# young-how/DQN-based-UAV-3D_path_planer

Hardware: NVIDIA H100
Metric: env steps/sec (+ DQN updates/sec), 500x500x100 city (higher is better)
Workload: dtype f64 env state / f32 obs+learner

## Files before the change

### dqn-based-uav-3d_path_planer_b200/csrc/learner.cu

```cuda
#include "learner.cuh"
#include "mlp_tile.cuh"
#include "tc_forward.cuh"

#include <math.h>
#include <string.h>

#include <string>
#include <vector>

namespace uavrl {

int build_mlp(int in_dim, int n_hidden, const int32_t *hidden, int head_main, int head_extra, NetDev &n)
{
    memset(&n, 0, sizeof(n));
    if (in_dim <= 0 || in_dim > kMaxDim) return fail(UAVRL_ERR_INVALID, "in_dim must be in [1,128]");
    if (n_hidden < 1 || n_hidden > UAVRL_MAX_HIDDEN) return fail(UAVRL_ERR_INVALID, "n_hidden must be in [1,4]");
    if (head_main < 1 || head_main + head_extra > 32) return fail(UAVRL_ERR_INVALID, "head width must be in [1,32]");
    n.in_dim = in_dim; n.n_actions = head_main; n.dueling = 0;
    n.n_layers = n_hidden + 1;
    int in = in_dim, poff = 0, soff = 0;
    for (int l = 0; l < n.n_layers; ++l) {
        LayerDev &L = n.L[l];
        const bool head = (l == n_hidden);
        const int out_real = head ? head_main : hidden[l];
// ... 522 lines not shown
        if (l->cfg.algo != UAVRL_ALGO_DQN) {
            a.img = l->tc_img_local; a.mode = kTcArgmax;
            if ((rc = launch_tc_forward(l, a, st))) return rc;
            a.mode = kTcTdGather;
        } else {
            a.mode = kTcTdMax;
        }
        a.img = l->tc_img_target;
        if ((rc = launch_tc_forward(l, a, st))) return rc;
        y_in = l->y_buf;
    }
    if (mid) UAVRL_CUDA(cudaEventRecord(mid[0], st));
    int nparts = grid, n_loss_parts = grid;
    AdamArgs a;
    memset(&a, 0, sizeof(a));
    a.P = l->net.P; a.apply = apply ? 1 : 0; a.world = l->world;
    a.img_floats = l->net.smem_w_floats; a.tc_floats = l->tc.train_img_bytes / 4;
    a.inv_b = 1.0f / (float)global_batch;
    if (apply && !partials_only) {
        adam_hyper(a, l->cfg.lr, ++l->adam_t);
        a.hard = hard_update_due(l);
    }
    if (y_in && l->tc_train_ok) {
        if (B > l->train_cap) {
            UAVRL_CUDA(cudaStreamSynchronize(st));
            cudaFree(l->act_buf); cudaFree(l->dz_buf);
            UAVRL_CUDA(cudaMalloc((void **)&l->act_buf, (size_t)l->G * B * (size_t)(l->tc.act_stride > 0 ? l->tc.act_stride : 4) * 4));
            UAVRL_CUDA(cudaMalloc((void **)&l->dz_buf, (size_t)l->G * B * (size_t)l->tc.dz_stride * 4));
            l->train_cap = B;
        }
        int rc = launch_tc_train(l, src, B, global_batch, y_in, &nparts, &n_loss_parts, st, mid ? mid[1] : nullptr, fuse_td);
        if (rc) return rc;
    } else {
    UpdateArgs ua;
    ua.img_local = l->img_local; ua.img_target = l->img_target; ua.partials = l->partials; ua.loss_partials = l->loss_partials;
    ua.B = B; ua.n_tiles = n_tiles; ua.algo = l->cfg.algo; ua.gamma = l->cfg.gamma; ua.dual = l->dual_weights;
    ua.loss_kind = l->cfg.loss_kind; ua.img_floats = l->net.smem_w_floats;
    ua.inv_global_b = 1.0f / (float)global_batch;
    ua.y_in = y_in;
    update_kernel<<<dim3(grid, l->G), kNetThreads, upd_smem_bytes(l->net, l->dual_weights), st>>>(l->net, src, ua);
    l->pdl_prev = kPdlNone;
    UAVRL_LAUNCHED();
    if (mid) UAVRL_CUDA(cudaEventRecord(mid[1], st));
    }
    if (mid) UAVRL_CUDA(cudaEventRecord(mid[2], st));
    l->last_nparts = nparts;
    l->last_n_loss_parts = n_loss_parts;
    l->last_global_batch = global_batch;
    if (partials_only) {
        if (per_batch) return per_set(l, B, l->per.idx, nullptr, l->per.abs_err, 1, st);
        return 0;
    }
    a.nparts = nparts; a.n_loss_parts = n_loss_parts;
// ... 454 lines not shown
```

### dqn-based-uav-3d_path_planer_b200/csrc/tc_chain.cuh

```cuda
#pragma once
#include "tc_forward.cuh"
#include "tma.cuh"
#include "wgmma.cuh"

namespace uavrl {

__device__ __forceinline__ void stage_trace(long long *t, int slot)
{
    if (t && blockIdx.x == 0 && blockIdx.y == 0 && threadIdx.x == 0) t[slot] = clock64();
}

template <class RowOf>
__device__ __forceinline__ void a0_load(const RowOf &row_of, int i0, int R, int in_dim, int K0, float4 (&v)[4])
{
    const int total = R * (K0 / 4), lgR = 31 - __clz(R);
#pragma unroll
    for (int u = 0; u < 4; ++u) {
        const int i = i0 + u * kTcThreads;
        const int r = i & (R - 1), j = i >> lgR;
        const float *rp = (i < total) ? row_of(r) : nullptr;
        v[u] = (rp && 4 * j < in_dim) ? __ldg(reinterpret_cast<const float4 *>(rp) + j) : make_float4(0.f, 0.f, 0.f, 0.f);
    }
}
__device__ __forceinline__ void a0_load_sel(const float *const *rows, const uint8_t *fresh, bool want_fresh, int R, int in_dim, int K0, float4 (&v)[4])
{
    const int total = R * (K0 / 4), lgR = 31 - __clz(R);
#pragma unroll
    for (int u = 0; u < 4; ++u) {
        const int i = threadIdx.x + u * kTcThreads;
        const int r = i & (R - 1), j = i >> lgR;
        const float *rp = (i < total) ? rows[r] : nullptr;
        const bool take = rp && 4 * j < in_dim && ((fresh[r] != 0) == want_fresh);
        if (!want_fresh) v[u] = take ? __ldg(reinterpret_cast<const float4 *>(rp) + j) : make_float4(0.f, 0.f, 0.f, 0.f);
        else if (take) v[u] = __ldcg(reinterpret_cast<const float4 *>(rp) + j);
    }
}
__device__ __forceinline__ void a0_store(const float4 (&v)[4], int i0, int R, int K0, unsigned char *Ahi, unsigned char *Alo)
{
    const int total = R * (K0 / 4), lgR = 31 - __clz(R);
    const uint32_t sbo = mma_sbo(K0);
#pragma unroll
    for (int u = 0; u < 4; ++u) {
        const int i = i0 + u * kTcThreads;
        if (i < total) {
            const int r = i & (R - 1), j = i >> lgR;
            float4 h, l;
            tf32_split(v[u].x, h.x, l.x); tf32_split(v[u].y, h.y, l.y); tf32_split(v[u].z, h.z, l.z); tf32_split(v[u].w, h.w, l.w);
            const uint32_t off = mma_off(r, 4 * j, sbo);
            *reinterpret_cast<float4 *>(Ahi + off) = h;
            *reinterpret_cast<float4 *>(Alo + off) = l;
        }
    }
}
template <class RowOf>
__device__ __forceinline__ void a0_gather(const RowOf &row_of, int R, int in_dim, int K0, unsigned char *Ahi, unsigned char *Alo)
{
    for (int i0 = threadIdx.x; i0 < R * (K0 / 4); i0 += 4 * kTcThreads) {
        float4 v[4];
        a0_load(row_of, i0, R, in_dim, K0, v);
        a0_store(v, i0, R, K0, Ahi, Alo);
    }
}

template <bool KEEP>
__device__ __forceinline__ uint32_t hidden_epilogue(const EpiSlice &e, const float *acc, int acc_ld, const float *bias, int N,
                                                    unsigned char *Ahi, unsigned char *Alo, float *act_row, bool mine)
{
    const uint32_t sbon = mma_sbo(N);
    uint32_t mk = 0u;
    for (int c = e.c0, sh = 0; c < N; c += e.step, sh += 4) {
        const float4 v = e.ld(acc, acc_ld, c);
        float4 x, h, lo4;
        x.x = fmaxf(v.x + bias[c + 0], 0.f); x.y = fmaxf(v.y + bias[c + 1], 0.f);
        x.z = fmaxf(v.z + bias[c + 2], 0.f); x.w = fmaxf(v.w + bias[c + 3], 0.f);
        tf32_split(x.x, h.x, lo4.x); tf32_split(x.y, h.y, lo4.y); tf32_split(x.z, h.z, lo4.z); tf32_split(x.w, h.w, lo4.w);
        const uint32_t off = mma_off(e.row, c, sbon);
        *reinterpret_cast<float4 *>(Ahi + off) = h;
        *reinterpret_cast<float4 *>(Alo + off) = lo4;
        if (KEEP) {
            if (mine) *reinterpret_cast<float4 *>(act_row + c) = x;
            mk |= ((x.x > 0.f ? 1u : 0u) | (x.y > 0.f ? 2u : 0u) | (x.z > 0.f ? 4u : 0u) | (x.w > 0.f ? 8u : 0u)) << sh;
        }
    }
    return mine ? mk : 0u;
}

template <bool DUELING>
__device__ __forceinline__ void q_combine(const float *bias, int nA, float (&q)[32])
{
#pragma unroll
    for (int j = 0; j < 32; ++j) q[j] += bias[j];
    if (DUELING) {
        float s = 0.f, V = 0.f;
#pragma unroll
        for (int j = 0; j < 32; ++j) { if (j < nA) s += q[j]; if (j == nA) V = q[j]; }
        const float mean = s / (float)nA;
#pragma unroll
        for (int j = 0; j < 32; ++j) q[j] = V + q[j] - mean;
    }
}
template <bool DUELING>
__device__ __forceinline__ void q_row(const float *acc, int acc_ld, int row, const float *bias, int nA, float (&q)[32])
{
// ... 7 lines not shown
#pragma unroll
    for (int j = 1; j < 32; ++j) if (j < nA && q[j] > bv) { bv = q[j]; best = j; }
    return best;
}
__device__ __forceinline__ float q_at(const float (&q)[32], int a)
{
    float v = 0.f;
#pragma unroll
    for (int j = 0; j < 32; ++j) if (j == a) v = q[j];
    return v;
}

__device__ __forceinline__ uint32_t fwd_image_split(const TcNet &tc) { return tc.n_layers > 1 ? (uint32_t)tc.L[1].hi_off : (uint32_t)tc.img_bytes; }
__device__ __forceinline__ void stage_forward_image(const TcNet &tc, unsigned char *W, const unsigned char *img, uint64_t *wbar, uint64_t *wbar2)
{
    const uint32_t split = fwd_image_split(tc);
    fence_proxy_async();
    bulk_g2s_chunked(W, img, split, wbar);
    if (split < (uint32_t)tc.img_bytes) bulk_g2s_chunked(W + split, img + split, (uint32_t)tc.img_bytes - split, wbar2);
}

template <bool FIXED, bool KEEP, class Mid, class Head, class Done>
__device__ __forceinline__ void forward_layers(const TcNet &tc, int R, const EpiSlice &e, unsigned char *Ahi, unsigned char *Alo,
                                               const unsigned char *W, float *acc, float *act_row, bool mine, Mid &&mid, Head &&head,
                                               Done &&done)
{
    const float *bias_all = reinterpret_cast<const float *>(W + tc.bias_base);
    for (int l = 0; l < tc.n_layers; ++l) {
        const TcLayer T = tc.L[l];
        mma_3xtf32<kMmaFwd, FIXED>(acc, tc.acc_ld, Ahi, Alo, W + T.hi_off, W + T.lo_off, mma_sbo(T.K_pad), T.N_pad, T.K_pad / 8, R);
        mid(l);
        const float *bias = bias_all + T.bias_off;
        if (l + 1 < tc.n_layers) {
            const uint32_t mk = hidden_epilogue<KEEP>(e, acc, tc.acc_ld, bias, T.N_pad, Ahi, Alo, KEEP ? act_row + tc.L[l + 1].act_off : nullptr, mine);
            fence_proxy_async();
            __syncthreads();
            done(l, mk);
        } else {
            head(l, bias);
        }
    }
}

}
```

### dqn-based-uav-3d_path_planer_b200/csrc/tc_forward.cu

```cuda
#include <stdarg.h>
#include <stdlib.h>
#include <string.h>

#include "tc_chain.cuh"

namespace uavrl {

static inline int rup(int x, int m) { return (x + m - 1) / m * m; }

size_t tc_smem_bytes(const TcNet &tc) { return (size_t)2 * tc.a_bytes + (size_t)tc.img_bytes + (size_t)tc.max_rows * tc.acc_ld * 4; }

int tc_build(const uavrl_learner_config &c, const NetDev &net, TcNet &tc, std::vector<int32_t> &hi_map, std::vector<int32_t> &lo_map,
             std::vector<int32_t> &hi2_map, std::vector<int32_t> &lo2_map)
{
    memset(&tc, 0, sizeof(tc));
    tc.n_layers = net.n_layers; tc.in_dim = net.in_dim; tc.n_actions = net.n_actions; tc.dueling = net.dueling;
    if (net.in_dim % 4 != 0) return -1;
    int off = 0, maxK = 0, k_pad = rup(net.in_dim, 8);
    for (int l = 0; l < net.n_layers; ++l) {
        const LayerDev &L = net.L[l];
        TcLayer &T = tc.L[l];
        const bool head = (l == net.n_layers - 1);
        T.K_real = L.in; T.K_pad = k_pad; T.N_real = L.out;
        T.N_pad = head ? 32 : rup(L.out, 16);
// ... 14 lines not shown
    for (int l = 0; l < net.n_layers; ++l) {
        TcLayer &T = tc.L[l];
        T.t_hi_off = T.t_lo_off = -1;
        if (l == 0) continue;
        const int bytes = T.K_pad * T.N_pad * 4;
        T.t_hi_off = toff; toff += bytes;
        T.t_lo_off = toff; toff += bytes;
    }
    tc.train_img_bytes = rup(toff, 16);
    tc.max_k = maxK;
    {
        int maxN = 32;
        for (int l = 0; l < net.n_layers; ++l) if (tc.L[l].N_pad > maxN) maxN = tc.L[l].N_pad;
        tc.acc_ld = rup(maxN, 32) + 4;
    }
    tc.max_rows = kTcTile;
    tc.a_bytes = (int)mma_tile_bytes(tc.max_rows, maxK);
    if (tc_smem_bytes(tc) + 4096 > 227 * 1024) {
        tc.max_rows = 64;
        tc.a_bytes = (int)mma_tile_bytes(tc.max_rows, maxK);
    }
    int ao = 0, dzo = 0;
    for (int l = 0; l < net.n_layers; ++l) {
        tc.L[l].act_off = (l == 0) ? -1 : ao;
        if (l > 0) ao += tc.L[l].K_pad;
        tc.L[l].dz_off = dzo; dzo += tc.L[l].N_pad;
    }
    tc.act_stride = ao; tc.dz_stride = dzo;
    hi_map.assign((size_t)net.P, -1); lo_map.assign((size_t)net.P, -1);
    hi2_map.assign((size_t)net.P, -1); lo2_map.assign((size_t)net.P, -1);
    auto elem = [](int k_pad_cols, int base, int n, int k) {
        const int sbo = (k_pad_cols / 4) * 128;
        return (base + (n >> 3) * sbo + (k >> 2) * 128 + (n & 7) * 16 + (k & 3) * 4) / 4;
    };
    for (int l = 0; l < net.n_layers; ++l) {
        const LayerDev &L = net.L[l];
        const TcLayer &T = tc.L[l];
        const int out_main = T.out_main;
        for (int o = 0; o < L.out; ++o) {
            const bool vrow = (o >= out_main);
            for (int k = 0; k < L.in; ++k) {
                const size_t pi = vrow ? (size_t)L.w2_off + (size_t)(o - out_main) * L.in + k : (size_t)L.w_off + (size_t)o * L.in + k;
                hi_map[pi] = elem(T.K_pad, T.hi_off, o, k);
                lo_map[pi] = elem(T.K_pad, T.lo_off, o, k);
                if (l > 0) {
                    hi2_map[pi] = elem(T.N_pad, T.t_hi_off, k, o);
                    lo2_map[pi] = elem(T.N_pad, T.t_lo_off, k, o);
                }
// ... 297 lines not shown
```

### dqn-based-uav-3d_path_planer_b200/csrc/tc_train.cu

```cuda
#include <string.h>
#include <stdlib.h>

#include <atomic>

#include "tc_chain.cuh"

namespace uavrl {

constexpr int kDwChunk = 128;

struct TcTrainArgs {
    const unsigned char *img;
    BatchSrc src;
    int32_t B, R, n_tiles;
    const float *y;
    float inv_global_b;
    float *act_buf, *dz_buf;
    float *loss_partials;
    int32_t loss_kind;
    int32_t fused_td, algo;
    float gamma;
    const unsigned char *img_target;
    int64_t img_stride;
    long long *trace;
};

struct TcDwArgs {
    BatchSrc src;
    int32_t B, n_chunks, P;
    int32_t n_slices;
    const float *act_buf, *dz_buf;
    float *partials;
    long long *trace;
};

template <int NPRE, bool DUELING, bool FIXED>
__global__ void __launch_bounds__(kTcThreads, 1) tc_train_kernel(TcNet tc, TcTrainArgs a)
{
    stage_trace(a.trace, 0);
    extern __shared__ __align__(1024) unsigned char smem[];
    const int R = a.R;
    const uint32_t a_bytes = (uint32_t)(R / 8) * mma_sbo(tc.max_k);
    unsigned char *Ahi = smem, *Alo = smem + a_bytes, *W = smem + 2 * a_bytes;
    float *acc = reinterpret_cast<float *>(W + tc.train_img_bytes);
    __shared__ uint64_t wbar, wbar2, wbar3;
    __shared__ const float *rows[kTcTile];
    __shared__ const float *rows2[kTcTile];
    __shared__ int s_act[kTcTile], s_astar[kTcTile];
    __shared__ uint8_t s_fresh[kTcTile];
    __shared__ float s_y[kTcTile], s_rew[kTcTile], s_done[kTcTile];
    __shared__ float s_loss[4];

    const int tid = threadIdx.x, warp = tid >> 5, lane = tid & 31, quad = warp & 3, half = warp >> 2;
    const int grp = blockIdx.y;
    const unsigned char *img = a.img + (size_t)grp * (size_t)a.img_stride, *img_t = a.img_target + (size_t)grp * (size_t)a.img_stride;
    const BatchSrc src = trainer_src(a.src, grp, a.B, tc.in_dim);
    const size_t r0 = (size_t)grp * (size_t)a.B;
    float *act_buf = a.act_buf + r0 * tc.act_stride, *dz_buf = a.dz_buf + r0 * tc.dz_stride;
    const float *y_in = a.y ? a.y + r0 : nullptr;
    constexpr int kCtl = kTcThreads - 32;
    if (tid == 0) s_loss[0] = s_loss[1] = s_loss[2] = s_loss[3] = 0.f;
    constexpr bool fused = NPRE > 0;
    constexpr int n_pre = NPRE;
    uint32_t wphase = 0;
    if (tid == kCtl) {
        mbar_init(&wbar, 1); mbar_init(&wbar2, 1); mbar_init(&wbar3, 1); fence_barrier_init();
        fence_proxy_async();
        if (!fused) bulk_g2s_chunked(W, img, (uint32_t)tc.train_img_bytes, &wbar);
        else {
            bulk_g2s_chunked(W, (n_pre == 2) ? img : img_t, (uint32_t)tc.img_bytes, &wbar);
            if (tc.train_img_bytes > tc.img_bytes)
                bulk_g2s_chunked(W + tc.img_bytes, img + tc.img_bytes, (uint32_t)(tc.train_img_bytes - tc.img_bytes), &wbar3);
        }
    }
    stage_trace(a.trace, 1);
    bool waited = false;

    uint32_t pkey[4];
    Philox::gen(src.key, src.epoch, 0x5A17ull, pkey);
    bool wready = false;
    const int nl = tc.n_layers;
    const int row = quad * 32 + lane;
    const bool live = quad * 32 < R;
    const EpiSlice e(R, kTcThreads);
    uint32_t hm1 = 0u, hm2 = 0u, hm3 = 0u, hm4 = 0u;
    const auto table = [](const float *const *t) { return [t](int r) { return t[r]; }; };

    for (int tile = blockIdx.x; tile < a.n_tiles; tile += gridDim.x) {
        const int base = tile * R;
        int64_t my_slot = -1;
        if (tid < R) {
            const int b = base + tid;
            const float *p = nullptr, *p2 = nullptr;
            bool fr = false;
            if (b < a.B) my_slot = resolve_rows(src, b, tc.in_dim, pkey, p, p2, &fr);
            rows[tid] = p;
            if (fused) { rows2[tid] = p2; s_astar[tid] = 0; s_fresh[tid] = fr ? 1 : 0; }
        }
        __syncthreads();
        const bool early_rows = n_pre > 0 && R * (tc.L[0].K_pad / 4) <= 4 * kTcThreads;
        float4 vmain[4], vnext[4];
        if (early_rows) {
            a0_load_sel(rows2, s_fresh, false, R, tc.in_dim, tc.L[0].K_pad, vnext);
            a0_load(table(rows), tid, R, tc.in_dim, tc.L[0].K_pad, vmain);
        }
        if (fused && !waited) { pdl_wait(); pdl_trigger(); waited = true; }
        int m_act = 0; float m_rew = 0.f, m_done = 0.f;
        if (my_slot >= 0) load_meta(src, my_slot, m_act, m_rew, m_done);
        if (early_rows) a0_load_sel(rows2, s_fresh, true, R, tc.in_dim, tc.L[0].K_pad, vnext);
        auto park_meta = [&]() { if (tid < R) { s_act[tid] = m_act; if (fused) { s_rew[tid] = m_rew; s_done[tid] = m_done; } } };
        stage_trace(a.trace, 2);
        for (int pass = 0; pass < n_pre; ++pass) {
// ... 5 lines not shown
            else a0_gather(table(rows2), R, tc.in_dim, tc.L[0].K_pad, Ahi, Alo);
            if (pass == 0) { park_meta(); stage_trace(a.trace, 3); }
            mbar_wait(&wbar, wphase); wphase ^= 1;
            fence_proxy_async();
            __syncthreads();
            if (pass == 0) stage_trace(a.trace, 4);
            const bool td_pass = (pass == n_pre - 1);
            const auto head = [&](int l, const float *bias) {
                if (half == 0 && live) {
                    float q[32], bv;
                    q_row<DUELING>(acc, tc.acc_ld, row, bias, tc.n_actions, q);
                    const int best = q_argmax(q, tc.n_actions, bv);
                    if (!td_pass) s_astar[row] = best;
                    else s_y[row] = td_target(s_rew[row], a.gamma, n_pre == 2 ? q_at(q, s_astar[row]) : bv, s_done[row]);
                }
                fence_proxy_async();
                __syncthreads();
                if (pass == 0) stage_trace(a.trace, 5 + l);
            };
            forward_layers<FIXED, false>(tc, R, e, Ahi, Alo, W, acc, nullptr, false, [](int) {}, head,
                                         [&](int l, uint32_t) { if (pass == 0) stage_trace(a.trace, 5 + l); });
        }
        if (fused && tid == kCtl) stage_forward_image(tc, W, img, &wbar, &wbar2);
        if (early_rows) a0_store(vmain, tid, R, tc.L[0].K_pad, Ahi, Alo);
        else a0_gather(table(rows), R, tc.in_dim, tc.L[0].K_pad, Ahi, Alo);
        stage_trace(a.trace, 9);
        if (!waited) { pdl_wait(); pdl_trigger(); waited = true; }
        if (n_pre == 0) park_meta();
        if (!fused && tid < R) s_y[tid] = (base + tid < a.B) ? y_in[base + tid] : 0.f;
        if (fused) { mbar_wait(&wbar, wphase); wphase ^= 1; }
        else if (!wready) { mbar_wait(&wbar, 0); wready = true; }
        fence_proxy_async();
        __syncthreads();
        stage_trace(a.trace, 10);
        const int gb = base + row;
        const bool mine = live && gb < a.B;
        const int egb = base + e.row;
        const bool emine = egb < a.B;

        const auto mid = [&](int l) {
            if (fused && l == 0 && fwd_image_split(tc) < (uint32_t)tc.img_bytes) mbar_wait(&wbar2, 0);
            if (l < 4) stage_trace(a.trace, 27 + l);
        };
        const auto head = [&](int l, const float *bias) {
            const TcLayer &T = tc.L[l];
            if (half == 0 && live) {
                const int nA = tc.n_actions;
                float q[32];
// ... 1 lines not shown
                stage_trace(a.trace, 21);
                q_combine<DUELING>(bias, nA, q);
                const int act = s_act[row];
                const float qa = q_at(q, act);
                stage_trace(a.trace, 22);
                float gq = 0.f, lterm = 0.f;
                if (mine) lterm = td_loss(src, gb, qa - s_y[row], a.loss_kind, a.inv_global_b, gq);
#pragma unroll
                for (int off = 16; off > 0; off >>= 1) lterm += __shfl_xor_sync(0xffffffffu, lterm, off);
                stage_trace(a.trace, 23);
                if (lane == 0) s_loss[quad] += lterm;
                stage_trace(a.trace, 24);
                float g[32];
                const float inv = 1.f / (float)nA;
#pragma unroll
                for (int j = 0; j < 32; ++j) {
                    float gj;
                    if (DUELING) gj = (j < nA) ? gq * ((j == act ? 1.f : 0.f) - inv) : (j == nA ? gq : 0.f);
                    else gj = (j == act) ? gq : 0.f;
                    g[j] = gj;
                }
                stage_trace(a.trace, 25);
                const uint32_t sbon = mma_sbo(T.N_pad);
                float *dz_row = dz_buf + (size_t)gb * tc.dz_stride + T.dz_off;
#pragma unroll
                for (int j = 0; j < 8; ++j) {
                    float4 x = make_float4(g[4 * j], g[4 * j + 1], g[4 * j + 2], g[4 * j + 3]), h, lo4;
                    tf32_split(x.x, h.x, lo4.x); tf32_split(x.y, h.y, lo4.y); tf32_split(x.z, h.z, lo4.z); tf32_split(x.w, h.w, lo4.w);
                    const uint32_t off = mma_off(row, 4 * j, sbon);
                    *reinterpret_cast<float4 *>(Ahi + off) = h;
                    *reinterpret_cast<float4 *>(Alo + off) = lo4;
                    if (mine) *reinterpret_cast<float4 *>(dz_row + 4 * j) = x;
                }
                stage_trace(a.trace, 26);
            }
            fence_proxy_async();
            __syncthreads();
            stage_trace(a.trace, 11 + l);
        };
        forward_layers<FIXED, true>(tc, R, e, Ahi, Alo, W, acc, act_buf + (size_t)egb * tc.act_stride, emine, mid, head,
                                    [&](int l, uint32_t mk) {
                                        if (l == 0) hm1 = mk; else if (l == 1) hm2 = mk; else if (l == 2) hm3 = mk; else hm4 = mk;
                                        stage_trace(a.trace, 11 + l);
                                    });

        if (fused && tc.train_img_bytes > tc.img_bytes) mbar_wait(&wbar3, 0);
        for (int l = nl - 1; l >= 1; --l) {
            const TcLayer T = tc.L[l];
            mma_3xtf32<kMmaDx, FIXED>(acc, tc.acc_ld, Ahi, Alo, W + T.t_hi_off, W + T.t_lo_off, mma_sbo(T.N_pad), T.K_pad, T.N_pad / 8, R);
            const uint32_t hmask = (l == 1) ? hm1 : (l == 2) ? hm2 : (l == 3) ? hm3 : hm4;
            const uint32_t sbon = mma_sbo(T.K_pad);
            float *dz_row = dz_buf + (size_t)egb * tc.dz_stride + tc.L[l - 1].dz_off;
            for (int c = e.c0, sh = 0; c < T.K_pad; c += e.step, sh += 4) {
                const float4 v = e.ld(acc, tc.acc_ld, c);
                const uint32_t m4 = hmask >> sh;
                float4 x, h, lo4;
                x.x = (m4 & 1u) ? v.x : 0.f; x.y = (m4 & 2u) ? v.y : 0.f;
                x.z = (m4 & 4u) ? v.z : 0.f; x.w = (m4 & 8u) ? v.w : 0.f;
                if (emine) *reinterpret_cast<float4 *>(dz_row + c) = x;
                if (l > 1) {
                    tf32_split(x.x, h.x, lo4.x); tf32_split(x.y, h.y, lo4.y); tf32_split(x.z, h.z, lo4.z); tf32_split(x.w, h.w, lo4.w);
                    const uint32_t off = mma_off(e.row, c, sbon);
                    *reinterpret_cast<float4 *>(Ahi + off) = h;
                    *reinterpret_cast<float4 *>(Alo + off) = lo4;
                }
            }
            fence_proxy_async();
            __syncthreads();
            stage_trace(a.trace, 16 + l);
        }
    }
    stage_trace(a.trace, 20);
    if (tid == 0) a.loss_partials[(size_t)grp * gridDim.x + blockIdx.x] = ((s_loss[0] + s_loss[1]) + s_loss[2]) + s_loss[3];
}

constexpr uint32_t kDwSbo = (kDwChunk / 4) * 128u + 16u;
constexpr int kDwARows = 128;

template <int LOG2F4, int U>
__device__ __forceinline__ void dw_load_rows(const float *const *rows, int width, float4 (&v)[U])
{
#pragma unroll
    for (int u = 0; u < U; ++u) {
        const int i = threadIdx.x + u * kTcThreads;
        const int b = i >> LOG2F4, jc = i & ((1 << LOG2F4) - 1);
        const float *r = (b < kDwChunk) ? rows[b] : nullptr;
        v[u] = (r && 4 * jc < width) ? __ldg(reinterpret_cast<const float4 *>(r) + jc) : make_float4(0.f, 0.f, 0.f, 0.f);
    }
}
template <int LOG2F4, int U>
__device__ __forceinline__ void dw_store_rows(const float4 (&v)[U], const float *const *rows, int ones_col, unsigned char *hi, unsigned char *lo)
{
#pragma unroll
    for (int u = 0; u < U; ++u) {
        const int i = threadIdx.x + u * kTcThreads;
        const int b = i >> LOG2F4, jc = i & ((1 << LOG2F4) - 1);
        if (b >= kDwChunk) continue;
        float4 x = v[u];
        if (ones_col >= 0 && (ones_col >> 2) == jc && rows[b]) x.x = 1.f;
        const float xs[4] = {x.x, x.y, x.z, x.w};
#pragma unroll
        for (int e = 0; e < 4; ++e) {
            float h, l;
            tf32_split(xs[e], h, l);
            const uint32_t off = mma_off(4 * jc + e, b, kDwSbo);
            *reinterpret_cast<float *>(hi + off) = h;
            *reinterpret_cast<float *>(lo + off) = l;
        }
    }
}

__global__ void __launch_bounds__(kTcThreads, 1) tc_dw_kernel(TcNet tc, TcDwArgs a)
{
    extern __shared__ __align__(1024) unsigned char smem[];
    const int l = blockIdx.x % tc.n_layers, slice = blockIdx.x / tc.n_layers;
    const int chunk = slice;
    const int grp = blockIdx.y;
    const BatchSrc src = trainer_src(a.src, grp, a.B, tc.in_dim);
    const float *act_buf = a.act_buf + (size_t)grp * a.B * tc.act_stride, *dz_buf = a.dz_buf + (size_t)grp * a.B * tc.dz_stride;
    const TcLayer T = tc.L[l];
    const int rowsA = T.K_real + 1;
    unsigned char *Ahi = smem, *Alo = Ahi + (kDwARows / 8) * kDwSbo, *Bhi = Alo + (kDwARows / 8) * kDwSbo;
    unsigned char *Blo = Bhi + (T.N_pad / 8) * kDwSbo;
    __shared__ const float *rows[2][kDwChunk];
    __shared__ const float *drows[2][kDwChunk];

    const int tid = threadIdx.x, warp = tid >> 5, lane = tid & 31, quad = warp & 3, half = warp >> 2;
    stage_trace(a.trace, 0);
    uint32_t pkey[4];
    Philox::gen(src.key, src.epoch, 0x5A17ull, pkey);
    auto resolve_chunk = [&](int c, int buf) {
        if (tid < kDwChunk) {
            const int b = c * kDwChunk + tid;
            const float *p = nullptr, *dzp = nullptr;
            if (c < a.n_chunks && b < a.B) {
                p = (l == 0) ? resolve_transition(src, b, tc.in_dim, pkey).s : act_buf + (size_t)b * tc.act_stride + T.act_off;
                dzp = dz_buf + (size_t)b * tc.dz_stride + T.dz_off;
            }
            rows[buf][tid] = p; drows[buf][tid] = dzp;
        }
    };
    resolve_chunk(slice, 0);
    __syncthreads();
    if (l != 0) { pdl_wait(); pdl_trigger(); }
    stage_trace(a.trace, 1);
    float4 va[16], vb[8];
    auto load_chunk = [&](int buf) {
        dw_load_rows<5, 16>(rows[buf], T.K_real, va);
        if (T.N_pad == 32) {
#pragma unroll
            for (int u = 4; u < 8; ++u) vb[u] = make_float4(0.f, 0.f, 0.f, 0.f);
            dw_load_rows<3, 4>(drows[buf], 32, reinterpret_cast<float4 (&)[4]>(vb));
        } else {
            dw_load_rows<4, 8>(drows[buf], 64, vb);
        }
    };
    if (l == 0) {
        dw_load_rows<5, 16>(rows[0], T.K_real, va);
        pdl_wait(); pdl_trigger();
        if (T.N_pad == 32) {
#pragma unroll
            for (int u = 4; u < 8; ++u) vb[u] = make_float4(0.f, 0.f, 0.f, 0.f);
            dw_load_rows<3, 4>(drows[0], 32, reinterpret_cast<float4 (&)[4]>(vb));
        } else {
            dw_load_rows<4, 8>(drows[0], 64, vb);
        }
    } else {
        load_chunk(0);
    }
    stage_trace(a.trace, 2);
    const int row0 = (tid >> 7) * 64;
    const bool wg_live = row0 < rowsA;
    float d[32];
    int it = 0;
    for (int c = slice; c < a.n_chunks; c += a.n_slices, ++it) {
        if (it > 0) __syncthreads();
        dw_store_rows<5, 16>(va, rows[it & 1], T.K_real, Ahi, Alo);
        if (T.N_pad == 32) dw_store_rows<3, 4>(reinterpret_cast<float4 (&)[4]>(vb), drows[it & 1], -1, Bhi, Blo);
        else dw_store_rows<4, 8>(vb, drows[it & 1], -1, Bhi, Blo);
        const int cn = c + a.n_slices;
        resolve_chunk(cn, (it + 1) & 1);
        fence_proxy_async();
        __syncthreads();
        stage_trace(a.trace, 4);
        if (cn < a.n_chunks) load_chunk((it + 1) & 1);
        if (wg_live) {
            const uint64_t ah = mma_desc(Ahi + (row0 / 8) * kDwSbo, kDwSbo), al = mma_desc(Alo + (row0 / 8) * kDwSbo, kDwSbo);
            const uint64_t bh = mma_desc(Bhi, kDwSbo), bl = mma_desc(Blo, kDwSbo);
            if (T.N_pad == 32) wgmma_3xtf32<32>(d, ah, al, bh, bl, kDwChunk / 8, it > 0 ? 1u : 0u);
            else wgmma_3xtf32<64>(d, ah, al, bh, bl, kDwChunk / 8, it > 0 ? 1u : 0u);
        }
    }
    stage_trace(a.trace, 5);
    __syncthreads();
    float *acc = reinterpret_cast<float *>(smem);
    const int acc_ld = T.N_pad + 4;
    if (wg_live) {
        if (T.N_pad == 32) store_frag<32>(d, acc, acc_ld, row0, 0, kDwARows);
        else store_frag<64>(d, acc, acc_ld, row0, 0, kDwARows);
    }
    __syncthreads();
    stage_trace(a.trace, 6);
    float *part = a.partials + ((size_t)grp * a.n_slices + chunk) * a.P;
    const int f = quad * 32 + lane;
    for (int c0 = half * 32; c0 < T.N_pad; c0 += 64) {
        if (quad * 32 >= rowsA) break;
        float v[32];
        acc_ld32(acc, acc_ld, f, c0, v);
        const int n_main = min(max(T.out_main - c0, 0), 32), n_all = min(max(T.N_real - c0, 0), 32);
        if (f > T.K_real) continue;
        const bool brow = (f == T.K_real);
        const int stride = brow ? 1 : T.K_real;
        const int i_main = brow ? T.b_off + c0 : T.w_off + f + c0 * T.K_real;
        const int i_val = brow ? T.b2_off + (c0 - T.out_main) : (T.w2_off >= 0 ? T.w2_off : 0) + f + (c0 - T.out_main) * T.K_real;
        float *p = part + i_main;
#pragma unroll
        for (int j = 0; j < 32; ++j) {
            if (j < n_main) *p = v[j];
            p += stride;
        }
        if (n_all > n_main) {
            float *q = part + i_val;
#pragma unroll
            for (int j = 0; j < 32; ++j) {
                if (j >= n_main && j < n_all) *q = v[j];
                q += stride;
            }
        }
    }
    stage_trace(a.trace, 7);
}

typedef void (*TrainKernel)(TcNet, TcTrainArgs);
template <int N, bool D>
static TrainKernel pick_train_x(bool fixed) { return fixed ? tc_train_kernel<N, D, true> : tc_train_kernel<N, D, false>; }
template <int N>
static TrainKernel pick_train_d(bool dueling, bool fixed) { return dueling ? pick_train_x<N, true>(fixed) : pick_train_x<N, false>(fixed); }
static TrainKernel pick_train_kernel(int npre, bool dueling, bool fixed)
{
    return npre == 0 ? pick_train_d<0>(dueling, fixed) : npre == 1 ? pick_train_d<1>(dueling, fixed) : pick_train_d<2>(dueling, fixed);
}

static size_t train_smem_bytes(const TcNet &tc, int R)
{
    return (size_t)2 * (R / 8) * mma_sbo(tc.max_k) + (size_t)tc.train_img_bytes + (size_t)R * tc.acc_ld * 4;
}
static size_t dw_smem_bytes(const TcNet &tc)
{
    int maxN = 32;
    for (int l = 0; l < tc.n_layers; ++l) if (tc.L[l].N_pad > maxN) maxN = tc.L[l].N_pad;
    return (size_t)2 * ((kDwARows + maxN) / 8) * kDwSbo;
}

int tc_train_init(uavrl_learner *l)
{
    l->tc_train_ok = false;
    TcNet &tc = l->tc;
    tc.train_max_rows = 0;
    for (int i = 0; i < tc.n_layers; ++i)
        if (tc.L[i].K_real + 1 > 128 || tc.L[i].K_real % 4 != 0 || (tc.L[i].N_pad != 32 && tc.L[i].N_pad != 64)) return 0;
    const bool fixed = tc_fixed_chains(tc, true);
    size_t train_static = 0, dw_static = 0;
    for (int np = 0; np < 3; ++np)
        for (int du = 0; du < 2; ++du) {
            cudaFuncAttributes fa;
            UAVRL_CUDA(cudaFuncGetAttributes(&fa, pick_train_kernel(np, du != 0, fixed)));
            if (fa.sharedSizeBytes > train_static) train_static = fa.sharedSizeBytes;
        }
    {
        cudaFuncAttributes fa;
        UAVRL_CUDA(cudaFuncGetAttributes(&fa, tc_dw_kernel));
        dw_static = fa.sharedSizeBytes;
    }
    const size_t train_budget = (size_t)227 * 1024 - train_static;
    if (train_smem_bytes(tc, 32) > train_budget || dw_smem_bytes(tc) + dw_static > (size_t)227 * 1024) return 0;
    if (train_smem_bytes(tc, 32) < (size_t)(32 / 8) * mma_sbo(tc.max_k) + (size_t)8 * mma_sbo(tc.max_k)) return 0;
    tc.train_max_rows = train_smem_bytes(tc, 64) <= train_budget ? 64 : 32;
    for (int np = 0; np < 3; ++np)
        for (int du = 0; du < 2; ++du)
            if (int rc = raise_dyn_smem(pick_train_kernel(np, du != 0, fixed), train_smem_bytes(tc, tc.train_max_rows))) return rc;
    if (int rc = raise_dyn_smem(tc_dw_kernel, dw_smem_bytes(tc))) return rc;
    const size_t cap = (size_t)l->cfg.batch_size, G = (size_t)l->G;
    UAVRL_CUDA(cudaMalloc((void **)&l->act_buf, G * cap * (size_t)(tc.act_stride > 0 ? tc.act_stride : 4) * 4));
    UAVRL_CUDA(cudaMalloc((void **)&l->dz_buf, G * cap * (size_t)tc.dz_stride * 4));
    l->train_cap = (int32_t)cap;
    l->tc_train_ok = true;
    return 0;
}

std::atomic<int> g_fuse_td{1};
int train_rows_per_tile(const TcNet &tc, int B)
{
    return (B > 32 * num_sms() && tc.train_max_rows == 64) ? 64 : 32;
}
bool tc_train_can_fuse_td(const uavrl_learner *l, int B)
{
    if (!g_fuse_td.load() || !l->tc_train_ok) return false;
    const int R = train_rows_per_tile(l->tc, B);
    return (B + R - 1) / R <= num_sms();
}
int launch_tc_train(uavrl_learner *l, const BatchSrc &src, int B, int global_batch, const float *y, int *n_grad_parts,
                    int *n_loss_parts, cudaStream_t st, cudaEvent_t after_chain, bool fused_td)
{
    const TcNet &tc = l->tc;
    TcTrainArgs a;
    memset(&a, 0, sizeof(a));
    a.img = l->tc_img_local; a.src = src; a.B = B; a.y = y; a.inv_global_b = 1.0f / (float)global_batch;
    a.act_buf = l->act_buf; a.dz_buf = l->dz_buf; a.loss_partials = l->loss_partials;
    a.loss_kind = l->cfg.loss_kind;
    a.fused_td = fused_td ? 1 : 0; a.algo = l->cfg.algo; a.gamma = l->cfg.gamma; a.img_target = l->tc_img_target;
    a.img_stride = tc.train_img_bytes;
    a.R = train_rows_per_tile(tc, B);
    a.n_tiles = (B + a.R - 1) / a.R;
    const int grid = a.n_tiles < num_sms() ? a.n_tiles : num_sms();
    const bool chain = l->pdl_chain && g_pdl.load();
    if (fused_td && a.n_tiles > grid) return fail(UAVRL_ERR_INVALID, "fused TD needs one tile per CTA");
    TcDwArgs d;
    memset(&d, 0, sizeof(d));
    if (int rc = stage_trace_alloc(&a.trace)) return rc;
    if (int rc = stage_trace_alloc(&d.trace)) { cudaFree(a.trace); return rc; }
    const bool use_pdl = chain && (fused_td ? (l->pdl_prev == kPdlEnv) : (l->pdl_prev == kPdlTd));
    const int npre = fused_td ? (l->cfg.algo != UAVRL_ALGO_DQN ? 2 : 1) : 0;
    UAVRL_CUDA(launch_kernel(pick_train_kernel(npre, tc.dueling != 0, tc_fixed_chains(tc, true)), dim3(grid, l->G), dim3(kTcThreads),
                             train_smem_bytes(tc, a.R), st, use_pdl, tc, a));
    l->pdl_prev = chain ? kPdlTrain : kPdlNone;
    UAVRL_LAUNCHED();
    if (after_chain) UAVRL_CUDA(cudaEventRecord(after_chain, st));
    d.src = src; d.B = B; d.n_chunks = (B + kDwChunk - 1) / kDwChunk; d.P = l->net.P;
    d.act_buf = l->act_buf; d.dz_buf = l->dz_buf; d.partials = l->partials;
    const int n_sm = num_sms();
    const int max_slices = n_sm / tc.n_layers > 0 ? n_sm / tc.n_layers : 1;
    d.n_slices = d.n_chunks < max_slices ? d.n_chunks : max_slices;
    const int dw_grid = d.n_slices * tc.n_layers;
    UAVRL_CUDA(launch_kernel(tc_dw_kernel, dim3(dw_grid, l->G), dim3(kTcThreads), dw_smem_bytes(tc), st, chain && !after_chain, tc, d));
    l->pdl_prev = chain ? kPdlDw : kPdlNone;
    UAVRL_LAUNCHED();
    const int rc_train = stage_trace_print(st, a.trace, "[train_trace] B=%d R=%d fused_td=%d", B, a.R, a.fused_td);
    const int rc_dw = stage_trace_print(st, d.trace, "[dw_trace] B=%d chunks=%d (CTA 0 = layer 0)", B, d.n_chunks);
    if (rc_train || rc_dw) return rc_train ? rc_train : rc_dw;
    *n_grad_parts = d.n_slices;
    *n_loss_parts = grid;
    return 0;
}

}

extern "C" int uavrl_set_fuse_dw_adam(int32_t on)
{
    return on ? uavrl::fail(UAVRL_ERR_INVALID, "uavrl_set_fuse_dw_adam: the fused weight-gradient + optimiser variant was removed") : 0;
}
extern "C" int uavrl_set_fuse_td(int32_t on) { uavrl::g_fuse_td.store(on ? 1 : 0); return 0; }
extern "C" int uavrl_learner_td_fused(const uavrl_learner *l, int32_t batch) { return (l && l->tc_ok && l->use_tc && uavrl::tc_train_can_fuse_td(l, batch)) ? 1 : 0; }
extern "C" int uavrl_learner_tc_route(const uavrl_learner *l, int32_t n, int32_t *out)
{
    if (!l || !out || n <= 0) return uavrl::fail(UAVRL_ERR_INVALID, "bad argument");
    const bool fwd = l->tc_ok && l->use_tc, train = fwd && l->tc_train_ok;
// ... 9 lines not shown
```

Baseline: 76.95 million.

## Store train scratch feature-major per chunk and split layer-0 weight-gradient work

The forward/backward training kernel now writes activations, including the layer-0 input rows, and dz values into chunk-major, feature-major scratch (feature × 128 samples). The dw kernel can then load contiguous float4 runs per feature instead of gathering rows through pointer tables and re-resolving replay transitions. Layer 0 optionally gets an extra CTA per slice covering input features above 64, so its larger K is split across two units. The trade is strided scalar stores in the training kernel and extra scratch memory for the stored inputs.

```diff
diff --git a/dqn-based-uav-3d_path_planer_b200/csrc/learner.cu b/dqn-based-uav-3d_path_planer_b200/csrc/learner.cu
--- a/dqn-based-uav-3d_path_planer_b200/csrc/learner.cu
+++ b/dqn-based-uav-3d_path_planer_b200/csrc/learner.cu
@@ -568,13 +568,6 @@
         a.hard = hard_update_due(l);
     }
     if (y_in && l->tc_train_ok) {
-        if (B > l->train_cap) {
-            UAVRL_CUDA(cudaStreamSynchronize(st));
-            cudaFree(l->act_buf); cudaFree(l->dz_buf);
-            UAVRL_CUDA(cudaMalloc((void **)&l->act_buf, (size_t)l->G * B * (size_t)(l->tc.act_stride > 0 ? l->tc.act_stride : 4) * 4));
-            UAVRL_CUDA(cudaMalloc((void **)&l->dz_buf, (size_t)l->G * B * (size_t)l->tc.dz_stride * 4));
-            l->train_cap = B;
-        }
         int rc = launch_tc_train(l, src, B, global_batch, y_in, &nparts, &n_loss_parts, st, mid ? mid[1] : nullptr, fuse_td);
         if (rc) return rc;
     } else {
diff --git a/dqn-based-uav-3d_path_planer_b200/csrc/tc_chain.cuh b/dqn-based-uav-3d_path_planer_b200/csrc/tc_chain.cuh
--- a/dqn-based-uav-3d_path_planer_b200/csrc/tc_chain.cuh
+++ b/dqn-based-uav-3d_path_planer_b200/csrc/tc_chain.cuh
@@ -8,6 +8,14 @@
 __device__ __forceinline__ void stage_trace(long long *t, int slot)
 {
     if (t && blockIdx.x == 0 && blockIdx.y == 0 && threadIdx.x == 0) t[slot] = clock64();
+}
+
+constexpr int kDwChunk = 128;
+template <class T>
+__host__ __device__ __forceinline__ T *dw_scratch(T *buf, int stride, int grp, int B, int b)
+{
+    const size_t n_chunks = (size_t)((B + kDwChunk - 1) / kDwChunk);
+    return buf + ((size_t)grp * n_chunks + (size_t)(b / kDwChunk)) * (size_t)stride * kDwChunk + (size_t)(b % kDwChunk);
 }
 
 template <class RowOf>
@@ -35,7 +43,8 @@
         else if (take) v[u] = __ldcg(reinterpret_cast<const float4 *>(rp) + j);
     }
 }
-__device__ __forceinline__ void a0_store(const float4 (&v)[4], int i0, int R, int K0, unsigned char *Ahi, unsigned char *Alo)
+__device__ __forceinline__ void a0_store(const float4 (&v)[4], int i0, int R, int K0, unsigned char *Ahi, unsigned char *Alo,
+                                         float *keep = nullptr)
 {
     const int total = R * (K0 / 4), lgR = 31 - __clz(R);
     const uint32_t sbo = mma_sbo(K0);
@@ -49,22 +58,27 @@
             const uint32_t off = mma_off(r, 4 * j, sbo);
             *reinterpret_cast<float4 *>(Ahi + off) = h;
             *reinterpret_cast<float4 *>(Alo + off) = l;
+            if (keep) {
+                float *k = keep + (size_t)(4 * j) * kDwChunk + r;
+                k[0] = v[u].x; k[kDwChunk] = v[u].y; k[2 * kDwChunk] = v[u].z; k[3 * kDwChunk] = v[u].w;
+            }
         }
     }
 }
 template <class RowOf>
-__device__ __forceinline__ void a0_gather(const RowOf &row_of, int R, int in_dim, int K0, unsigned char *Ahi, unsigned char *Alo)
+__device__ __forceinline__ void a0_gather(const RowOf &row_of, int R, int in_dim, int K0, unsigned char *Ahi, unsigned char *Alo,
+                                          float *keep = nullptr)
 {
     for (int i0 = threadIdx.x; i0 < R * (K0 / 4); i0 += 4 * kTcThreads) {
         float4 v[4];
         a0_load(row_of, i0, R, in_dim, K0, v);
-        a0_store(v, i0, R, K0, Ahi, Alo);
+        a0_store(v, i0, R, K0, Ahi, Alo, keep);
     }
 }
 
 template <bool KEEP>
 __device__ __forceinline__ uint32_t hidden_epilogue(const EpiSlice &e, const float *acc, int acc_ld, const float *bias, int N,
-                                                    unsigned char *Ahi, unsigned char *Alo, float *act_row, bool mine)
+                                                    unsigned char *Ahi, unsigned char *Alo, float *act_col, bool mine)
 {
     const uint32_t sbon = mma_sbo(N);
     uint32_t mk = 0u;
@@ -78,7 +92,10 @@
         *reinterpret_cast<float4 *>(Ahi + off) = h;
         *reinterpret_cast<float4 *>(Alo + off) = lo4;
         if (KEEP) {
-            if (mine) *reinterpret_cast<float4 *>(act_row + c) = x;
+            if (mine) {
+                float *p = act_col + (size_t)c * kDwChunk;
+                p[0] = x.x; p[kDwChunk] = x.y; p[2 * kDwChunk] = x.z; p[3 * kDwChunk] = x.w;
+            }
             mk |= ((x.x > 0.f ? 1u : 0u) | (x.y > 0.f ? 2u : 0u) | (x.z > 0.f ? 4u : 0u) | (x.w > 0.f ? 8u : 0u)) << sh;
         }
     }
@@ -132,7 +149,7 @@
 
 template <bool FIXED, bool KEEP, class Mid, class Head, class Done>
 __device__ __forceinline__ void forward_layers(const TcNet &tc, int R, const EpiSlice &e, unsigned char *Ahi, unsigned char *Alo,
-                                               const unsigned char *W, float *acc, float *act_row, bool mine, Mid &&mid, Head &&head,
+                                               const unsigned char *W, float *acc, float *act_col, bool mine, Mid &&mid, Head &&head,
                                                Done &&done)
 {
     const float *bias_all = reinterpret_cast<const float *>(W + tc.bias_base);
@@ -142,7 +159,8 @@
         mid(l);
         const float *bias = bias_all + T.bias_off;
         if (l + 1 < tc.n_layers) {
-            const uint32_t mk = hidden_epilogue<KEEP>(e, acc, tc.acc_ld, bias, T.N_pad, Ahi, Alo, KEEP ? act_row + tc.L[l + 1].act_off : nullptr, mine);
+            const uint32_t mk = hidden_epilogue<KEEP>(e, acc, tc.acc_ld, bias, T.N_pad, Ahi, Alo,
+                                                      KEEP ? act_col + (size_t)tc.L[l + 1].act_off * kDwChunk : nullptr, mine);
             fence_proxy_async();
             __syncthreads();
             done(l, mk);
diff --git a/dqn-based-uav-3d_path_planer_b200/csrc/tc_forward.cu b/dqn-based-uav-3d_path_planer_b200/csrc/tc_forward.cu
--- a/dqn-based-uav-3d_path_planer_b200/csrc/tc_forward.cu
+++ b/dqn-based-uav-3d_path_planer_b200/csrc/tc_forward.cu
@@ -60,8 +60,7 @@
     }
     int ao = 0, dzo = 0;
     for (int l = 0; l < net.n_layers; ++l) {
-        tc.L[l].act_off = (l == 0) ? -1 : ao;
-        if (l > 0) ao += tc.L[l].K_pad;
+        tc.L[l].act_off = ao; ao += tc.L[l].K_pad;
         tc.L[l].dz_off = dzo; dzo += tc.L[l].N_pad;
     }
     tc.act_stride = ao; tc.dz_stride = dzo;
diff --git a/dqn-based-uav-3d_path_planer_b200/csrc/tc_train.cu b/dqn-based-uav-3d_path_planer_b200/csrc/tc_train.cu
--- a/dqn-based-uav-3d_path_planer_b200/csrc/tc_train.cu
+++ b/dqn-based-uav-3d_path_planer_b200/csrc/tc_train.cu
@@ -6,8 +6,6 @@
 #include "tc_chain.cuh"
 
 namespace uavrl {
-
-constexpr int kDwChunk = 128;
 
 struct TcTrainArgs {
     const unsigned char *img;
@@ -26,9 +24,9 @@
 };
 
 struct TcDwArgs {
-    BatchSrc src;
     int32_t B, n_chunks, P;
     int32_t n_slices;
+    int32_t split0;
     const float *act_buf, *dz_buf;
     float *partials;
     long long *trace;
@@ -55,9 +53,7 @@
     const int grp = blockIdx.y;
     const unsigned char *img = a.img + (size_t)grp * (size_t)a.img_stride, *img_t = a.img_target + (size_t)grp * (size_t)a.img_stride;
     const BatchSrc src = trainer_src(a.src, grp, a.B, tc.in_dim);
-    const size_t r0 = (size_t)grp * (size_t)a.B;
-    float *act_buf = a.act_buf + r0 * tc.act_stride, *dz_buf = a.dz_buf + r0 * tc.dz_stride;
-    const float *y_in = a.y ? a.y + r0 : nullptr;
+    const float *y_in = a.y ? a.y + (size_t)grp * (size_t)a.B : nullptr;
     constexpr int kCtl = kTcThreads - 32;
     if (tid == 0) s_loss[0] = s_loss[1] = s_loss[2] = s_loss[3] = 0.f;
     constexpr bool fused = NPRE > 0;
@@ -88,6 +84,7 @@
 
     for (int tile = blockIdx.x; tile < a.n_tiles; tile += gridDim.x) {
         const int base = tile * R;
+        float *act_t = dw_scratch(a.act_buf, tc.act_stride, grp, a.B, base), *dz_t = dw_scratch(a.dz_buf, tc.dz_stride, grp, a.B, base);
         int64_t my_slot = -1;
         if (tid < R) {
             const int b = base + tid;
@@ -139,8 +136,9 @@
                                          [&](int l, uint32_t) { if (pass == 0) stage_trace(a.trace, 5 + l); });
         }
         if (fused && tid == kCtl) stage_forward_image(tc, W, img, &wbar, &wbar2);
-        if (early_rows) a0_store(vmain, tid, R, tc.L[0].K_pad, Ahi, Alo);
-        else a0_gather(table(rows), R, tc.in_dim, tc.L[0].K_pad, Ahi, Alo);
+        float *s_keep = act_t + (size_t)tc.L[0].act_off * kDwChunk;
+        if (early_rows) a0_store(vmain, tid, R, tc.L[0].K_pad, Ahi, Alo, s_keep);
+        else a0_gather(table(rows), R, tc.in_dim, tc.L[0].K_pad, Ahi, Alo, s_keep);
         stage_trace(a.trace, 9);
         if (!waited) { pdl_wait(); pdl_trigger(); waited = true; }
         if (n_pre == 0) park_meta();
@@ -188,7 +186,7 @@
                 }
                 stage_trace(a.trace, 25);
                 const uint32_t sbon = mma_sbo(T.N_pad);
-                float *dz_row = dz_buf + (size_t)gb * tc.dz_stride + T.dz_off;
+                float *dz_col = dz_t + row + (size_t)T.dz_off * kDwChunk;
 #pragma unroll
                 for (int j = 0; j < 8; ++j) {
                     float4 x = make_float4(g[4 * j], g[4 * j + 1], g[4 * j + 2], g[4 * j + 3]), h, lo4;
@@ -196,7 +194,10 @@
                     const uint32_t off = mma_off(row, 4 * j, sbon);
                     *reinterpret_cast<float4 *>(Ahi + off) = h;
                     *reinterpret_cast<float4 *>(Alo + off) = lo4;
-                    if (mine) *reinterpret_cast<float4 *>(dz_row + 4 * j) = x;
+                    if (mine) {
+                        float *p = dz_col + (size_t)(4 * j) * kDwChunk;
+                        p[0] = x.x; p[kDwChunk] = x.y; p[2 * kDwChunk] = x.z; p[3 * kDwChunk] = x.w;
+                    }
                 }
                 stage_trace(a.trace, 26);
             }
@@ -204,7 +205,7 @@
             __syncthreads();
             stage_trace(a.trace, 11 + l);
         };
-        forward_layers<FIXED, true>(tc, R, e, Ahi, Alo, W, acc, act_buf + (size_t)egb * tc.act_stride, emine, mid, head,
+        forward_layers<FIXED, true>(tc, R, e, Ahi, Alo, W, acc, act_t + e.row, emine, mid, head,
                                     [&](int l, uint32_t mk) {
                                         if (l == 0) hm1 = mk; else if (l == 1) hm2 = mk; else if (l == 2) hm3 = mk; else hm4 = mk;
                                         stage_trace(a.trace, 11 + l);
@@ -216,14 +217,17 @@
             mma_3xtf32<kMmaDx, FIXED>(acc, tc.acc_ld, Ahi, Alo, W + T.t_hi_off, W + T.t_lo_off, mma_sbo(T.N_pad), T.K_pad, T.N_pad / 8, R);
             const uint32_t hmask = (l == 1) ? hm1 : (l == 2) ? hm2 : (l == 3) ? hm3 : hm4;
             const uint32_t sbon = mma_sbo(T.K_pad);
-            float *dz_row = dz_buf + (size_t)egb * tc.dz_stride + tc.L[l - 1].dz_off;
+            float *dz_col = dz_t + e.row + (size_t)tc.L[l - 1].dz_off * kDwChunk;
             for (int c = e.c0, sh = 0; c < T.K_pad; c += e.step, sh += 4) {
                 const float4 v = e.ld(acc, tc.acc_ld, c);
                 const uint32_t m4 = hmask >> sh;
                 float4 x, h, lo4;
                 x.x = (m4 & 1u) ? v.x : 0.f; x.y = (m4 & 2u) ? v.y : 0.f;
                 x.z = (m4 & 4u) ? v.z : 0.f; x.w = (m4 & 8u) ? v.w : 0.f;
-                if (emine) *reinterpret_cast<float4 *>(dz_row + c) = x;
+                if (emine) {
+                    float *p = dz_col + (size_t)c * kDwChunk;
+                    p[0] = x.x; p[kDwChunk] = x.y; p[2 * kDwChunk] = x.z; p[3 * kDwChunk] = x.w;
+                }
                 if (l > 1) {
                     tf32_split(x.x, h.x, lo4.x); tf32_split(x.y, h.y, lo4.y); tf32_split(x.z, h.z, lo4.z); tf32_split(x.w, h.w, lo4.w);
                     const uint32_t off = mma_off(e.row, c, sbon);
@@ -240,116 +244,91 @@
     if (tid == 0) a.loss_partials[(size_t)grp * gridDim.x + blockIdx.x] = ((s_loss[0] + s_loss[1]) + s_loss[2]) + s_loss[3];
 }
 
-constexpr uint32_t kDwSbo = (kDwChunk / 4) * 128u + 16u;
+constexpr uint32_t kDwSbo = (kDwChunk / 4) * 128u;
 constexpr int kDwARows = 128;
-
-template <int LOG2F4, int U>
-__device__ __forceinline__ void dw_load_rows(const float *const *rows, int width, float4 (&v)[U])
-{
+static_assert(kTcThreads == 8 * (kDwChunk / 4), "dw_load / dw_store: 8 features x kDwChunk / 4 sample groups per pass");
+
+template <int U>
+__device__ __forceinline__ void dw_load(const float *blk, int lo, int width, int n_valid, float4 (&v)[U])
+{
+    const int f0 = threadIdx.x & 7, s4 = 4 * (threadIdx.x >> 3);
 #pragma unroll
     for (int u = 0; u < U; ++u) {
-        const int i = threadIdx.x + u * kTcThreads;
-        const int b = i >> LOG2F4, jc = i & ((1 << LOG2F4) - 1);
-        const float *r = (b < kDwChunk) ? rows[b] : nullptr;
-        v[u] = (r && 4 * jc < width) ? __ldg(reinterpret_cast<const float4 *>(r) + jc) : make_float4(0.f, 0.f, 0.f, 0.f);
-    }
-}
-template <int LOG2F4, int U>
-__device__ __forceinline__ void dw_store_rows(const float4 (&v)[U], const float *const *rows, int ones_col, unsigned char *hi, unsigned char *lo)
-{
+        const int f = 8 * u + f0;
+        v[u] = (f >= lo && f < width && s4 < n_valid) ? __ldg(reinterpret_cast<const float4 *>(blk + (size_t)f * kDwChunk + s4))
+                                           : make_float4(0.f, 0.f, 0.f, 0.f);
+    }
+}
+template <int U>
+__device__ __forceinline__ void dw_store(const float4 (&v)[U], int f_lo, int f_hi, int n_valid, int ones_row, unsigned char *hi,
+                                         unsigned char *lo)
+{
+    const int f0 = threadIdx.x & 7, s4 = 4 * (threadIdx.x >> 3);
 #pragma unroll
     for (int u = 0; u < U; ++u) {
-        const int i = threadIdx.x + u * kTcThreads;
-        const int b = i >> LOG2F4, jc = i & ((1 << LOG2F4) - 1);
-        if (b >= kDwChunk) continue;
-        float4 x = v[u];
-        if (ones_col >= 0 && (ones_col >> 2) == jc && rows[b]) x.x = 1.f;
-        const float xs[4] = {x.x, x.y, x.z, x.w};
-#pragma unroll
-        for (int e = 0; e < 4; ++e) {
-            float h, l;
-            tf32_split(xs[e], h, l);
-            const uint32_t off = mma_off(4 * jc + e, b, kDwSbo);
-            *reinterpret_cast<float *>(hi + off) = h;
-            *reinterpret_cast<float *>(lo + off) = l;
-        }
+        const int f = 8 * u + f0;
+        if (f < f_lo || f >= f_hi) continue;
+        float4 x = (f == ones_row) ? make_float4(1.f, 1.f, 1.f, 1.f) : v[u];
+        if (s4 + 4 > n_valid) {
+            x.x = s4 < n_valid ? x.x : 0.f; x.y = s4 + 1 < n_valid ? x.y : 0.f;
+            x.z = s4 + 2 < n_valid ? x.z : 0.f; x.w = s4 + 3 < n_valid ? x.w : 0.f;
+        }
+        float4 h, lo4;
+        tf32_split(x.x, h.x, lo4.x); tf32_split(x.y, h.y, lo4.y); tf32_split(x.z, h.z, lo4.z); tf32_split(x.w, h.w, lo4.w);
+        const uint32_t off = mma_off(f, s4, kDwSbo);
+        *reinterpret_cast<float4 *>(hi + off) = h;
+        *reinterpret_cast<float4 *>(lo + off) = lo4;
     }
 }
 
 __global__ void __launch_bounds__(kTcThreads, 1) tc_dw_kernel(TcNet tc, TcDwArgs a)
 {
     extern __shared__ __align__(1024) unsigned char smem[];
-    const int l = blockIdx.x % tc.n_layers, slice = blockIdx.x / tc.n_layers;
+    const int n_units = tc.n_layers + a.split0;
+    const int unit = blockIdx.x % n_units, slice = blockIdx.x / n_units;
+    const int l = unit < tc.n_layers ? unit : 0;
+    const int f_lo = unit == tc.n_layers ? 64 : 0, f_hi = (a.split0 && unit == 0) ? 64 : kDwARows;
     const int chunk = slice;
     const int grp = blockIdx.y;
-    const BatchSrc src = trainer_src(a.src, grp, a.B, tc.in_dim);
-    const float *act_buf = a.act_buf + (size_t)grp * a.B * tc.act_stride, *dz_buf = a.dz_buf + (size_t)grp * a.B * tc.dz_stride;
     const TcLayer T = tc.L[l];
     const int rowsA = T.K_real + 1;
     unsigned char *Ahi = smem, *Alo = Ahi + (kDwARows / 8) * kDwSbo, *Bhi = Alo + (kDwARows / 8) * kDwSbo;
     unsigned char *Blo = Bhi + (T.N_pad / 8) * kDwSbo;
-    __shared__ const float *rows[2][kDwChunk];
-    __shared__ const float *drows[2][kDwChunk];
 
     const int tid = threadIdx.x, warp = tid >> 5, lane = tid & 31, quad = warp & 3, half = warp >> 2;
     stage_trace(a.trace, 0);
-    uint32_t pkey[4];
-    Philox::gen(src.key, src.epoch, 0x5A17ull, pkey);
-    auto resolve_chunk = [&](int c, int buf) {
-        if (tid < kDwChunk) {
-            const int b = c * kDwChunk + tid;
-            const float *p = nullptr, *dzp = nullptr;
-            if (c < a.n_chunks && b < a.B) {
-                p = (l == 0) ? resolve_transition(src, b, tc.in_dim, pkey).s : act_buf + (size_t)b * tc.act_stride + T.act_off;
-                dzp = dz_buf + (size_t)b * tc.dz_stride + T.dz_off;
-            }
-            rows[buf][tid] = p; drows[buf][tid] = dzp;
-        }
-    };
-    resolve_chunk(slice, 0);
-    __syncthreads();
-    if (l != 0) { pdl_wait(); pdl_trigger(); }
+    pdl_wait(); pdl_trigger();
     stage_trace(a.trace, 1);
     float4 va[16], vb[8];
-    auto load_chunk = [&](int buf) {
-        dw_load_rows<5, 16>(rows[buf], T.K_real, va);
+    auto load_chunk = [&](int c) {
+        const int nv = a.B - c * kDwChunk;
+        dw_load<16>(dw_scratch(a.act_buf, tc.act_stride, grp, a.B, c * kDwChunk) + (size_t)T.act_off * kDwChunk, f_lo,
+                    min(T.K_real, f_hi), nv, va);
+        const float *dz = dw_scratch(a.dz_buf, tc.dz_stride, grp, a.B, c * kDwChunk) + (size_t)T.dz_off * kDwChunk;
         if (T.N_pad == 32) {
 #pragma unroll
             for (int u = 4; u < 8; ++u) vb[u] = make_float4(0.f, 0.f, 0.f, 0.f);
-            dw_load_rows<3, 4>(drows[buf], 32, reinterpret_cast<float4 (&)[4]>(vb));
+            dw_load<4>(dz, 0, 32, nv, reinterpret_cast<float4 (&)[4]>(vb));
         } else {
-            dw_load_rows<4, 8>(drows[buf], 64, vb);
+            dw_load<8>(dz, 0, 64, nv, vb);
         }
     };
-    if (l == 0) {
-        dw_load_rows<5, 16>(rows[0], T.K_real, va);
-        pdl_wait(); pdl_trigger();
-        if (T.N_pad == 32) {
-#pragma unroll
-            for (int u = 4; u < 8; ++u) vb[u] = make_float4(0.f, 0.f, 0.f, 0.f);
-            dw_load_rows<3, 4>(drows[0], 32, reinterpret_cast<float4 (&)[4]>(vb));
-        } else {
-            dw_load_rows<4, 8>(drows[0], 64, vb);
-        }
-    } else {
-        load_chunk(0);
-    }
+    load_chunk(slice);
     stage_trace(a.trace, 2);
     const int row0 = (tid >> 7) * 64;
-    const bool wg_live = row0 < rowsA;
+    const bool wg_live = row0 < rowsA && row0 >= f_lo && row0 < f_hi;
     float d[32];
     int it = 0;
     for (int c = slice; c < a.n_chunks; c += a.n_slices, ++it) {
         if (it > 0) __syncthreads();
-        dw_store_rows<5, 16>(va, rows[it & 1], T.K_real, Ahi, Alo);
-        if (T.N_pad == 32) dw_store_rows<3, 4>(reinterpret_cast<float4 (&)[4]>(vb), drows[it & 1], -1, Bhi, Blo);
-        else dw_store_rows<4, 8>(vb, drows[it & 1], -1, Bhi, Blo);
-        const int cn = c + a.n_slices;
-        resolve_chunk(cn, (it + 1) & 1);
+        const int nv = a.B - c * kDwChunk;
+        dw_store<16>(va, f_lo, f_hi, nv, T.K_real, Ahi, Alo);
+        if (T.N_pad == 32) dw_store<4>(reinterpret_cast<float4 (&)[4]>(vb), 0, 32, nv, -1, Bhi, Blo);
+        else dw_store<8>(vb, 0, 64, nv, -1, Bhi, Blo);
         fence_proxy_async();
         __syncthreads();
         stage_trace(a.trace, 4);
-        if (cn < a.n_chunks) load_chunk((it + 1) & 1);
+        if (c + a.n_slices < a.n_chunks) load_chunk(c + a.n_slices);
         if (wg_live) {
             const uint64_t ah = mma_desc(Ahi + (row0 / 8) * kDwSbo, kDwSbo), al = mma_desc(Alo + (row0 / 8) * kDwSbo, kDwSbo);
             const uint64_t bh = mma_desc(Bhi, kDwSbo), bl = mma_desc(Blo, kDwSbo);
@@ -370,7 +349,7 @@
     float *part = a.partials + ((size_t)grp * a.n_slices + chunk) * a.P;
     const int f = quad * 32 + lane;
     for (int c0 = half * 32; c0 < T.N_pad; c0 += 64) {
-        if (quad * 32 >= rowsA) break;
+        if (quad * 32 >= rowsA || quad * 32 < f_lo || quad * 32 >= f_hi) break;
         float v[32];
         acc_ld32(acc, acc_ld, f, c0, v);
         const int n_main = min(max(T.out_main - c0, 0), 32), n_all = min(max(T.N_real - c0, 0), 32);
@@ -416,6 +395,17 @@
     int maxN = 32;
     for (int l = 0; l < tc.n_layers; ++l) if (tc.L[l].N_pad > maxN) maxN = tc.L[l].N_pad;
     return (size_t)2 * ((kDwARows + maxN) / 8) * kDwSbo;
+}
+static int alloc_train_scratch(uavrl_learner *l, int B)
+{
+    const size_t samples = (size_t)l->G * (size_t)((B + kDwChunk - 1) / kDwChunk) * kDwChunk;
+    cudaFree(l->act_buf); cudaFree(l->dz_buf);
+    l->act_buf = l->dz_buf = nullptr;
+    l->train_cap = 0;
+    UAVRL_CUDA(cudaMalloc((void **)&l->act_buf, samples * (size_t)l->tc.act_stride * 4));
+    UAVRL_CUDA(cudaMalloc((void **)&l->dz_buf, samples * (size_t)l->tc.dz_stride * 4));
+    l->train_cap = B;
+    return 0;
 }
 
 int tc_train_init(uavrl_learner *l)
@@ -446,10 +436,7 @@
         for (int du = 0; du < 2; ++du)
             if (int rc = raise_dyn_smem(pick_train_kernel(np, du != 0, fixed), train_smem_bytes(tc, tc.train_max_rows))) return rc;
     if (int rc = raise_dyn_smem(tc_dw_kernel, dw_smem_bytes(tc))) return rc;
-    const size_t cap = (size_t)l->cfg.batch_size, G = (size_t)l->G;
-    UAVRL_CUDA(cudaMalloc((void **)&l->act_buf, G * cap * (size_t)(tc.act_stride > 0 ? tc.act_stride : 4) * 4));
-    UAVRL_CUDA(cudaMalloc((void **)&l->dz_buf, G * cap * (size_t)tc.dz_stride * 4));
-    l->train_cap = (int32_t)cap;
+    if (int rc = alloc_train_scratch(l, l->cfg.batch_size)) return rc;
     l->tc_train_ok = true;
     return 0;
 }
@@ -469,6 +456,10 @@
                     int *n_loss_parts, cudaStream_t st, cudaEvent_t after_chain, bool fused_td)
 {
     const TcNet &tc = l->tc;
+    if (B > l->train_cap) {
+        UAVRL_CUDA(cudaStreamSynchronize(st));
+        if (int rc = alloc_train_scratch(l, B)) return rc;
+    }
     TcTrainArgs a;
     memset(&a, 0, sizeof(a));
     a.img = l->tc_img_local; a.src = src; a.B = B; a.y = y; a.inv_global_b = 1.0f / (float)global_batch;
@@ -492,12 +483,13 @@
     l->pdl_prev = chain ? kPdlTrain : kPdlNone;
     UAVRL_LAUNCHED();
     if (after_chain) UAVRL_CUDA(cudaEventRecord(after_chain, st));
-    d.src = src; d.B = B; d.n_chunks = (B + kDwChunk - 1) / kDwChunk; d.P = l->net.P;
+    d.B = B; d.n_chunks = (B + kDwChunk - 1) / kDwChunk; d.P = l->net.P;
     d.act_buf = l->act_buf; d.dz_buf = l->dz_buf; d.partials = l->partials;
     const int n_sm = num_sms();
     const int max_slices = n_sm / tc.n_layers > 0 ? n_sm / tc.n_layers : 1;
     d.n_slices = d.n_chunks < max_slices ? d.n_chunks : max_slices;
-    const int dw_grid = d.n_slices * tc.n_layers;
+    d.split0 = (tc.L[0].K_real + 1 > 64 && d.n_slices * (tc.n_layers + 1) <= n_sm) ? 1 : 0;
+    const int dw_grid = d.n_slices * (tc.n_layers + d.split0);
     UAVRL_CUDA(launch_kernel(tc_dw_kernel, dim3(dw_grid, l->G), dim3(kTcThreads), dw_smem_bytes(tc), st, chain && !after_chain, tc, d));
     l->pdl_prev = chain ? kPdlDw : kPdlNone;
     UAVRL_LAUNCHED();
```

After: 82.61 million, median of 6. +7.4%, better.
